# fransiskusbudi/multimodal_segmentation_project

Hardware: AMD Instinct MI355X
Metric: 3D volumes/sec (96^3, 4-class) fwd+bwd per node (higher is better)
Workload: dtype bf16; 1 GPU; UNet3D(1->4, features 16/32/64/128) 96^3 patch, per-GPU batch 2, fwd + Dice/CE loss + bwd + AdamW + metrics, dropout 0.0; global_batch=2, parallelism=dp1, hipgraph=False

## Files before the change

include/mi3d.h:

```cpp
#ifndef MI3D_H
#define MI3D_H
#include <stddef.h>
#include <stdint.h>

#ifdef __cplusplus
extern "C" {
#endif

#define MI3D_DTYPE_F32 0
#define MI3D_DTYPE_BF16 1
#define MI3D_MAX_LEVELS 6

const char* mi3d_last_error(void);
int mi3d_abi_version(void);

typedef struct mi3d_unet_desc {
    int32_t in_channels, out_channels;
    int32_t n_levels;
    int32_t features[MI3D_MAX_LEVELS];
    int32_t N, D, H, W;
    int32_t dtype;
    float bn_momentum, bn_eps;
} mi3d_unet_desc;

// ... 149 lines not shown
                 void* workspace, size_t workspace_bytes, void* stream);
int mi3d_fill_boxes_i64(int64_t* label, int C, int D, int H, int W, int n_holes, const int32_t* hole_lo,
                        const int32_t* hole_size, int64_t fill, void* stream);

size_t mi3d_conv3_workspace_bytes(int Cin, int Cout, int N, int D, int H, int W);
int mi3d_conv3_forward(int in_dtype, int out_dtype, const void* x, int xcs, int Cin, const float* w, const float* bias,
                       void* y, int ycs, int Cout, int N, int D, int H, int W, void* workspace, size_t workspace_bytes,
                       void* stream);
int mi3d_conv3_backward(int x_dtype, int dy_dtype, const void* x, int xcs, int Cin, const float* w, const void* dy,
                        int dycs, int Cout, void* dx, int dxcs, float* dW, float* db, int accumulate, int N, int D,
                        int H, int W, void* workspace, size_t workspace_bytes, void* stream);
size_t mi3d_bn_workspace_bytes(int C);
int mi3d_bn_relu_drop_forward(int dtype, const void* y, int ycs, int C, int64_t M, int64_t V, const float* gamma,
                              const float* beta, float* running_mean, float* running_var, int64_t* num_batches_tracked,
                              float momentum, float eps, int training, const float* drop, void* z, int zcs, float* stat,
                              void* workspace, void* stream);
int mi3d_bn_relu_drop_backward(int dtype, const void* dz, int dzcs, const void* y, int ycs, int C, int64_t M, int64_t V,
                               const float* stat, const float* drop, void* dy, int dycs, float* dgamma, float* dbeta,
                               int accumulate, void* workspace, void* stream);
int mi3d_bn_relu_drop_pool_forward(int dtype, const void* y, int ycs, int C, int N, int D, int H, int W, const float* gamma,
                                   const float* beta, float* running_mean, float* running_var, int64_t* num_batches_tracked,
                                   float momentum, float eps, const float* drop, void* z, int zcs, void* pooled, int pcs,
                                   float* stat, void* workspace, void* stream);
int mi3d_maxpool2_forward(int dtype, const void* z, int zcs, int C, int N, int D, int H, int W, void* p, int pcs,
                          void* stream);
int mi3d_maxpool2_backward(int dtype, const void* dp, int dpcs, const void* z, int zcs, const void* dskip, int dskipcs,
                           void* dz, int dzcs, int C, int N, int D, int H, int W, void* stream);
size_t mi3d_upconv2_workspace_bytes(int Cin, int Cout, int N, int D, int H, int W);
int mi3d_upconv2_forward(int dtype, const void* x, int xcs, int Cin, const float* w, const float* bias, void* y, int ycs,
                         int Cout, int N, int D, int H, int W, void* workspace, size_t workspace_bytes, void* stream);
int mi3d_upconv2_backward(int dtype, const void* x, int xcs, int Cin, const float* w, const void* gy, int gycs, int Cout,
                          void* dx, int dxcs, float* dW, float* db, int accumulate, int N, int D, int H, int W,
                          void* workspace, size_t workspace_bytes, void* stream);
size_t mi3d_conv1_workspace_bytes(int Cin, int Cout);
int mi3d_conv1_forward(int dtype, const void* z, int zcs, int Cin, const float* w, const float* bias, float* logits, int Cout,
                       int N, int64_t V, void* stream);
int mi3d_conv1_backward(int dtype, const void* z, int zcs, int Cin, const float* w, const float* dlogits, int Cout, void* dz,
                        int dzcs, float* dW, float* db, int accumulate, int N, int64_t V, void* workspace,
                        size_t workspace_bytes, void* stream);
int mi3d_ncdhw_to_ndhwc(int dtype, const float* src, void* dst, int dcs, int C, int N, int64_t V, void* stream);
int mi3d_ndhwc_to_ncdhw(int dtype, const void* src, int scs, float* dst, int C, int N, int64_t V, void* stream);

int mi3d_graph_begin(void* stream);
int mi3d_graph_end(void* stream, void** graph_exec_out);
int mi3d_graph_launch(void* graph_exec, void* stream);
int mi3d_graph_destroy(void* graph_exec);
// ... 6 lines not shown
```

multimodal_segmentation_project_amd/_lib.py:

```python
import contextlib
import ctypes as C
import os

import torch

_HERE = os.path.dirname(os.path.abspath(__file__))
LIB_PATH = os.environ.get("MI3D_LIB_PATH") or os.path.join(_HERE, "libmi3d.so")
MAX_LEVELS = 6
LOSS_COEF_FLOATS = 20
DTYPE_F32, DTYPE_BF16 = 0, 1

vp, i32, i64, f32, sz = C.c_void_p, C.c_int, C.c_int64, C.c_float, C.c_size_t


class UNetDesc(C.Structure):
    _fields_ = [("in_channels", C.c_int32), ("out_channels", C.c_int32), ("n_levels", C.c_int32),
                ("features", C.c_int32 * MAX_LEVELS), ("N", C.c_int32), ("D", C.c_int32), ("H", C.c_int32),
                ("W", C.c_int32), ("dtype", C.c_int32), ("bn_momentum", C.c_float), ("bn_eps", C.c_float)]


class LossCfg(C.Structure):
    _fields_ = [("w_ce", C.c_float), ("region_kind", C.c_int32), ("w_reg", C.c_float), ("alpha", C.c_float),
                ("beta", C.c_float), ("eps", C.c_float), ("w_kd", C.c_float), ("temperature", C.c_float)]

# ... 73 lines not shown
    "mi3d_preprocess_mri": (i32, [vp, vp, i64, f32, f32, vp, vp]),
    "mi3d_remap_labels": (i32, [vp, vp, i64, i32, vp]),
    "mi3d_zoom3_workspace_bytes": (sz, [i32, i32, i32]),
    "mi3d_zoom3_cubic": (i32, [vp, vp, i32, i32, i32, i32, i32, i32, vp, i32, vp, i32, vp, i32, i32, f32, f32, vp]),
    "mi3d_zoom3_nearest_i64": (i32, [vp, vp, i32, i32, i32, i32, i32, i32, vp, i32, vp, i32, vp, i32, vp]),
    "mi3d_reorient3": (i32, [vp, i32, vp, i32, i32, i32, i32, i64, i64, i64, i32, vp]),
    "mi3d_zoom3_cubic_src": (i32, [vp, i32, i64, i64, i64, vp, i32, i32, i32, i32, i32, i32, vp, i32, vp, i32, vp, i32, i32, f32, f32, vp]),
    "mi3d_zoom3_nearest_src": (i32, [vp, i32, i64, i64, i64, vp, i32, i32, i32, i32, i32, i32, vp, i32, vp, i32, vp, i32, vp]),
    "mi3d_merge_masks3": (i32, [_MP, i32, i64, i64, i64, vp, i32, i32, i32, i32, i32, i32, vp, i32, vp, i32, vp, i32, vp]),
    "mi3d_plane_affine": (i32, [vp, vp, vp, vp, i32, i32, i32, i32, i32, i32, C.POINTER(C.c_double), C.POINTER(C.c_double), i32, vp]),
    "mi3d_augment_workspace_bytes": (sz, []),
    "mi3d_augment": (i32, [vp, vp, vp, i32, i32, i32, i32, _AP, vp, sz, vp]),
    "mi3d_fill_boxes_i64": (i32, [vp, i32, i32, i32, i32, i32, C.POINTER(C.c_int32), C.POINTER(C.c_int32), i64, vp]),
    "mi3d_conv3_workspace_bytes": (sz, [i32, i32, i32, i32, i32, i32]),
    "mi3d_conv3_forward": (i32, [i32, i32, vp, i32, i32, vp, vp, vp, i32, i32, i32, i32, i32, i32, vp, sz, vp]),
    "mi3d_conv3_backward": (i32, [i32, i32, vp, i32, i32, vp, vp, i32, i32, vp, i32, vp, vp, i32, i32, i32, i32, i32,
                                  vp, sz, vp]),
    "mi3d_bn_workspace_bytes": (sz, [i32]),
    "mi3d_bn_relu_drop_forward": (i32, [i32, vp, i32, i32, i64, i64, vp, vp, vp, vp, vp, f32, f32, i32, vp, vp, i32,
                                        vp, vp, vp]),
    "mi3d_bn_relu_drop_backward": (i32, [i32, vp, i32, vp, i32, i32, i64, i64, vp, vp, vp, i32, vp, vp, i32, vp, vp]),
    "mi3d_bn_relu_drop_pool_forward": (i32, [i32, vp, i32, i32, i32, i32, i32, i32, vp, vp, vp, vp, vp, f32, f32, vp, vp, i32,
                                             vp, i32, vp, vp, vp]),
    "mi3d_conv1_workspace_bytes": (sz, [i32, i32]),
    "mi3d_conv1_forward": (i32, [i32, vp, i32, i32, vp, vp, vp, i32, i32, i64, vp]),
    "mi3d_conv1_backward": (i32, [i32, vp, i32, i32, vp, vp, i32, vp, i32, vp, vp, i32, i32, i64, vp, sz, vp]),
    "mi3d_maxpool2_forward": (i32, [i32, vp, i32, i32, i32, i32, i32, i32, vp, i32, vp]),
    "mi3d_maxpool2_backward": (i32, [i32, vp, i32, vp, i32, vp, i32, vp, i32, i32, i32, i32, i32, i32, vp]),
    "mi3d_upconv2_workspace_bytes": (sz, [i32, i32, i32, i32, i32, i32]),
    "mi3d_upconv2_forward": (i32, [i32, vp, i32, i32, vp, vp, vp, i32, i32, i32, i32, i32, i32, vp, sz, vp]),
    "mi3d_upconv2_backward": (i32, [i32, vp, i32, i32, vp, vp, i32, i32, vp, i32, vp, vp, i32, i32, i32, i32, i32, vp,
                                    sz, vp]),
    "mi3d_ncdhw_to_ndhwc": (i32, [i32, vp, vp, i32, i32, i32, i64, vp]),
    "mi3d_ndhwc_to_ncdhw": (i32, [i32, vp, i32, vp, i32, i32, i64, vp]),
    "mi3d_graph_begin": (i32, [vp]),
    "mi3d_graph_end": (i32, [vp, C.POINTER(vp)]),
    "mi3d_graph_launch": (i32, [vp, vp]),
    "mi3d_graph_destroy": (i32, [vp]),
}

_lib = None


class Mi3dError(RuntimeError):
    pass

# ... 82 lines not shown
```

multimodal_segmentation_project_amd/csrc/api.hip:

```cpp
#include "../../include/mi3d.h"
#include <stdlib.h>
#include <string.h>

#include "ops.h"

static_assert(MI3D_LOSS_COEF_FLOATS >= 2 * MI3D_MAX_CLASSES + 4, "coef buffer too small");

namespace {
struct RouteEntry { const char* name; int Mi3dRoutes::*field; };
const RouteEntry ROUTE_TABLE[] = {
#define MI3D_ROUTE_ENTRY(name, dflt) {#name, &Mi3dRoutes::name},
    MI3D_ROUTE_LIST(MI3D_ROUTE_ENTRY)
#undef MI3D_ROUTE_ENTRY
};
constexpr int N_ROUTES = sizeof(ROUTE_TABLE) / sizeof(ROUTE_TABLE[0]);
Mi3dRoutes load_routes() {
    Mi3dRoutes r;
    for (int i = 0; i < N_ROUTES; i++) {
        char env[64] = "MI3D_";
        size_t n = 5;
        for (const char* c = ROUTE_TABLE[i].name; *c && n + 1 < sizeof(env); c++) env[n++] = (*c >= 'a' && *c <= 'z') ? *c - 32 : *c;
        env[n] = 0;
        const char* v = getenv(env);
        if (!v) continue;
// ... 183 lines not shown
    BnSmall sm{(const float*)workspace, small_rows, gamma, beta, running_mean, running_var, num_batches_tracked, momentum, eps};
    return bn_apply_relu_drop(dtype, y, ycs, C, M, V, stat, drop, z, zcs, s, small_rows > 0 ? &sm : nullptr);
}
int mi3d_bn_relu_drop_backward(int dtype, const void* dz, int dzcs, const void* y, int ycs, int C, int64_t M, int64_t V,
                               const float* stat, const float* drop, void* dy, int dycs, float* dgamma, float* dbeta,
                               int accumulate, void* workspace, void* stream) {
    MI3D_CHECK_ARG(dz && y && stat && dy && workspace, "mi3d_bn_relu_drop_backward: null pointer");
    return bn_bwd(dtype, dz, dzcs, y, ycs, C, M, V, stat, drop, dy, dycs, dgamma, dbeta, accumulate, (float*)workspace,
                  (hipStream_t)stream);
}
int mi3d_bn_relu_drop_pool_forward(int dtype, const void* y, int ycs, int C, int N, int D, int H, int W, const float* gamma,
                                   const float* beta, float* running_mean, float* running_var, int64_t* num_batches_tracked,
                                   float momentum, float eps, const float* drop, void* z, int zcs, void* pooled, int pcs,
                                   float* stat, void* workspace, void* stream) {
    MI3D_CHECK_ARG(y && gamma && beta && z && pooled && stat && workspace, "mi3d_bn_relu_drop_pool_forward: null pointer");
    hipStream_t s = (hipStream_t)stream;
    Geo g{N, D, H, W};
    int small_rows = 0;
    MI3D_TRY(bn_train_stats(dtype, y, ycs, C, g.M(), gamma, beta, running_mean, running_var, num_batches_tracked, momentum, eps,
                            stat, (float*)workspace, s, &small_rows));
    BnSmall sm{(const float*)workspace, small_rows, gamma, beta, running_mean, running_var, num_batches_tracked, momentum, eps};
    return bn_apply_relu_drop_pool(dtype, y, ycs, C, g, stat, drop, z, zcs, pooled, pcs, s, small_rows > 0 ? &sm : nullptr);
}
size_t mi3d_conv1_workspace_bytes(int Cin, int Cout) { return conv1_bwd_ws_floats(Cin, Cout) * sizeof(float); }
int mi3d_conv1_forward(int dtype, const void* z, int zcs, int Cin, const float* w, const float* bias, float* logits, int Cout,
                       int N, int64_t V, void* stream) {
    MI3D_CHECK_ARG(z && w && logits, "mi3d_conv1_forward: null pointer");
    MI3D_CHECK_ARG(dtype == MI3D_F32 || dtype == MI3D_BF16, "mi3d_conv1_forward: bad dtype %d", dtype);
    return conv1_fwd(dtype, z, zcs, Cin, w, bias, logits, Cout, N, V, (hipStream_t)stream);
}
int mi3d_head_loss_supported(int dtype, int Cin, int C, const mi3d_loss_cfg* cfg) {
    return cfg && head_loss_bwd_ok(dtype, nullptr, Cin, Cin, C, to_cfg(cfg), nullptr, Cin) ? 1 : 0;
}
int mi3d_head_loss_forward(const void* z, int zcs, int Cin, const float* w, const float* bias, const int64_t* labels,
                           const float* teacher, int N, int C, int D, int64_t V, const mi3d_loss_cfg* cfg, float* loss_out, float* coef,
                           float* metrics_out, void* loss_workspace, void* metrics_workspace, float* logits_opt, void* stream) {
    MI3D_CHECK_ARG(z && w && labels && cfg && loss_out && coef && loss_workspace, "mi3d_head_loss_forward: null pointer");
    return head_loss_fwd(z, zcs, Cin, w, bias, labels, teacher, N, C, V, to_cfg(cfg), loss_out, coef, loss_workspace, (hipStream_t)stream,
                         D, metrics_out, metrics_workspace, logits_opt);
}
int mi3d_head_loss_backward(const void* z, int zcs, int Cin, const float* w, const float* bias, const int64_t* labels,
                            const float* teacher, int N, int C, int64_t V, const mi3d_loss_cfg* cfg, const float* coef,
                            const float* grad_scale, void* dz, int dzcs, float* dW, float* db, int accumulate, void* workspace,
                            size_t workspace_bytes, void* stream) {
    MI3D_CHECK_ARG(z && w && labels && cfg && coef && dz && workspace, "mi3d_head_loss_backward: null pointer");
    MI3D_CHECK_ARG(workspace_bytes >= mi3d_conv1_workspace_bytes(Cin, C), "mi3d_head_loss_backward: workspace too small");
// ... 149 lines not shown
```

multimodal_segmentation_project_amd/csrc/bn.hip:

```cpp
#include "ops.h"

namespace {

constexpr int BLK = 256;
constexpr int MAXBLK = 1024;
constexpr int FIN_T = 256;

template <int VEC> __device__ __forceinline__ bool row_map(int C, int& r, int& g, int& R) {
    int G = C / VEC;
    R = BLK / G;
    r = threadIdx.x / G;
    g = threadIdx.x - r * G;
    return r < R;
}

template <int VEC, int K> __device__ __forceinline__ void block_colreduce(const float (&acc)[K][VEC], int C, int r, int g, int R,
                                                                           bool active, float* lds, float* part) {
    if (active) {
#pragma unroll
        for (int k = 0; k < K; k++)
#pragma unroll
            for (int i = 0; i < VEC; i++) lds[((k * R + r) * C) + g * VEC + i] = acc[k][i];
    }
    __syncthreads();
// ... 197 lines not shown
        int c = threadIdx.x;
        if (c < C) {
            BnCoef k = bn_coef(sq[0], sq[1], t.M, t.gamma[c], t.beta[c], t.eps);
            ab[c] = k.a;
            ab[MAXC_BN + c] = k.b;
            if (blockIdx.x == 0)
                bn_publish(k, c, C, t.M, stat, t.running_mean, t.running_var, t.num_batches_tracked, t.momentum);
        }
        __syncthreads();
#pragma unroll
        for (int i = 0; i < VEC; i++) { a[i] = ab[g * VEC + i]; b[i] = ab[MAXC_BN + g * VEC + i]; }
    } else {
#pragma unroll
        for (int i = 0; i < VEC; i++) { a[i] = stat[2 * C + g * VEC + i]; b[i] = stat[3 * C + g * VEC + i]; }
    }
}

__device__ __forceinline__ float bn_act(float v, float a, float b, float s) {
    float t = fmaf(v, a, b);
    t = t > 0.f ? t : 0.f;
    return t * s;
}
__device__ __forceinline__ float bn_mask(float v, float a, float b, float s) { return fmaf(v, a, b) > 0.f ? s : 0.f; }

__global__ void bn_eval_stats_kernel(int C, const float* gamma, const float* beta, const float* rm,
                                     const float* rv, float eps, float* stat) {
    int c = blockIdx.x * blockDim.x + threadIdx.x;
    if (c >= C) return;
    double inv = 1.0 / sqrt((double)rv[c] + (double)eps);
    stat[c] = rm[c];
    stat[C + c] = (float)inv;
    stat[2 * C + c] = (float)((double)gamma[c] * inv);
    stat[3 * C + c] = (float)((double)beta[c] - (double)rm[c] * (double)gamma[c] * inv);
}

template <int VEC>
struct DropCache {
    float s[VEC];
    int64_t bound = 0;
    int smp = -1;
    __device__ __forceinline__ DropCache() {
#pragma unroll
        for (int i = 0; i < VEC; i++) s[i] = 1.f;
    }
    __device__ __forceinline__ void at(const float* __restrict__ drop, int64_t row, int64_t V, int C, int c0) {
        if (drop && row >= bound) {
// ... 312 lines not shown
        c2o = MAXC_BN;
    }
#pragma unroll
    for (int i = 0; i < VEC; i++) {
        int c = g * VEC + i;
        float mean = stat[c], inv = stat[C + c];
        a[i] = stat[2 * C + c]; b[i] = stat[3 * C + c];
        gg[i] = SMALL ? a[i] : coef[2 * C + c];
        bwd_coef(c12[c], c12[c2o + c], gg[i], mean, inv, A[i], B[i]);
    }
    DropCache<VEC> dc;
    for (; row < M; row += rstep) {
        float yv[VEC], gv[VEC], o[VEC];
        ldv<T, VEC>(y + row * ycs + g * VEC, yv);
        ldv<T, VEC>(dz + row * dzcs + g * VEC, gv);
        dc.at(drop, row, V, C, g * VEC);
#pragma unroll
        for (int i = 0; i < VEC; i++)
            o[i] = fmaf(gg[i] * bn_mask(yv[i], a[i], b[i], dc.s[i]), gv[i], fmaf(A[i], yv[i], B[i]));
        stv<T, VEC>(dy + row * dycs + g * VEC, o);
    }
}

__global__ void bn_fold_all_kernel(BnFoldJobs J) {
    const BnFoldJob& j = J.j[blockIdx.x];
    for (int c = threadIdx.x; c < j.C; c += blockDim.x) {
        double a = (double)j.gamma[c] / sqrt((double)j.rv[c] + (double)J.eps);
        j.scale[c] = (float)a;
        j.fbias[c] = (float)(((double)(j.conv_bias ? j.conv_bias[c] : 0.f) - (double)j.rm[c]) * a + (double)j.beta[c]);
    }
}

__global__ void bn_deferred_apply_kernel(BnDeferJobs J) {
    const BnDeferJob& j = J.j[blockIdx.x];
    for (int c = threadIdx.x; c < j.C; c += blockDim.x) {
        j.rm[c] = (float)((1.0 - J.momentum) * j.rm[c] + J.momentum * j.side[c]);
        j.rv[c] = (float)((1.0 - J.momentum) * j.rv[c] + J.momentum * j.side[j.C + c]);
    }
    if (threadIdx.x == 0 && j.nbt) *j.nbt += 1;
}

inline bool vec8_ok(int C, int cs_a, int cs_b, const void* pa, const void* pb, int esz) {
    return C % 8 == 0 && cs_a % 8 == 0 && cs_b % 8 == 0 && ((uintptr_t)pa % 16 == 0) && ((uintptr_t)pb % 16 == 0) &&
           (C / 8) <= BLK && esz > 0;
}

// ... 128 lines not shown
    DISPATCH_T(dtype, T, {
        bool v8 = vec8_ok(C, ycs, zcs, y, z, sizeof(T)) && pcs % 8 == 0 && ((uintptr_t)pooled % 16 == 0);
        int grid = v8 ? stream_grid(M / 8 * (C / 8), C / 8) : stream_grid(M / 8 * C, C);
        const T* yp = (const T*)y; T* zp = (T*)z; T* pp = (T*)pooled;
        const int G8 = C / 8;
        const bool pair = v8 && (G8 & (G8 - 1)) == 0 && G8 <= 32 && !mi3d_routes().no_pool_pair;
        if (pair) grid = stream_grid(M / 8 * G8 * 2, G8 * 2);
        if (small && small->nrows > SMALL_ROWS) {
            if (pair && dtype == MI3D_BF16 && wide_rows_ok(C, small->nrows)) {
                bn_apply_pool_wide_kernel<<<wide_grid(M / 8 * G8 * 2), WNT, 0, s>>>((const bf16*)y, ycs, C, g.N, g.D, g.H, g.W, stat, t, drop, (bf16*)z, zcs, (bf16*)pooled, pcs);
                MI3D_LAUNCH_CHECK();
                return 0;
            }
            MI3D_CHECK_ARG(small->nrows <= SMALL_ROWS, "bn_apply_pool: %d partial rows need the wide kernel (C = %d)", small->nrows, C);
        }
        DISPATCH_VEC(v8, VEC, DISPATCH_FLAG(small != nullptr, TRAIN, DISPATCH_FLAG(pair, PAIR, {
            bn_apply_pool_kernel<T, VEC, TRAIN, PAIR && VEC == 8><<<grid, BLK, 0, s>>>(yp, ycs, C, g.N, g.D, g.H, g.W, stat, t, drop, zp, zcs, pp, pcs);
        });););
        MI3D_LAUNCH_CHECK();
    });
    return 0;
}

int bn_bwd(int dtype, const void* dz, int dzcs, const void* y, int ycs, int C, int64_t M, int64_t V,
           const float* stat, const float* drop, void* dy, int dycs, float* dgamma, float* dbeta, int accumulate,
           float* ws, hipStream_t s, const SlabJob* extra, const float* skp, int ks, const SlabJob* extra2) {
    MI3D_CHECK_ARG(C >= 1 && C <= BLK && M >= 1, "bn_bwd: bad C=%d", C);
    MI3D_CHECK_ARG(!drop || M < (1ll << 32), "bn_bwd: dropout path needs M < 2^32 (32-bit sample index)");
    float* part = ws;
    float* coef = ws + (size_t)MAXBLK * 2 * C;
    bool small = bn_small(C, M);
    DISPATCH_T(dtype, T, {
        bool v8 = vec8_ok(C, ycs, dzcs, y, dz, sizeof(T)) && dycs % 8 == 0 && ((uintptr_t)dy % 16 == 0);
        MI3D_CHECK_ARG(!skp || (v8 && ks >= 1), "bn_bwd: split-K source needs the vector path");
        int G = v8 ? C / 8 : C, R = BLK / G;
        int nblk = reduce_grid(M, R);
        if (small) nblk = bn_small_rows(nblk);
        size_t lds = (size_t)2 * R * C * sizeof(float);
        const T* dzp = (const T*)dz; const T* yp = (const T*)y; T* dyp = (T*)dy;
        if (extra && extra->nblocks > 0) {
            SlabJob j2 = (extra2 && extra2->nblocks > 0) ? *extra2 : SlabJob();
            int tot = nblk + extra->nblocks + j2.nblocks;
            DISPATCH_VEC(v8, VEC, {
                bn_bwd_reduce_slab_kernel<T, VEC><<<tot, BLK, lds, s>>>(nblk, dzp, dzcs, yp, ycs, C, M, V, stat, drop, part, *extra, j2, skp, ks);
            });
        } else
            DISPATCH_VEC(v8, VEC, { bn_bwd_reduce_kernel<T, VEC><<<nblk, BLK, lds, s>>>(dzp, dzcs, yp, ycs, C, M, V, stat, drop, part, skp, ks); });
        MI3D_LAUNCH_CHECK();
        if (!small) {
            bn_bwd_finalize_kernel<<<C, FIN_T, 0, s>>>(part, nblk, C, M, stat, dgamma, dbeta, accumulate, coef);
            MI3D_LAUNCH_CHECK();
// ... 43 lines not shown
```

multimodal_segmentation_project_amd/csrc/ops.h:

```cpp
#pragma once
#include "common.h"
#include "slab_sum.h"

struct Geo {
    int N, D, H, W;
    int64_t V() const { return (int64_t)D * H * W; }
    int64_t M() const { return (int64_t)N * D * H * W; }
};

size_t conv3_direct_pack_floats(int Cin, int Cout);
int conv3_direct_pack(const float* w, int Cin, int Cout, float* wp_fwd, float* wp_dgrad, hipStream_t s,
                      const float* scale = nullptr);
int conv3_direct_fwd(int in_dtype, int out_dtype, const void* x, int xcs, int Cin, const float* wp,
                     const float* bias, void* y, int ycs, int Cout, Geo g, hipStream_t s, int relu = 0);
size_t conv3_direct_wgrad_ws_floats(int Cin, int Cout, Geo g);
int conv3_direct_wgrad(int x_dtype, int dy_dtype, const void* x, int xcs, int Cin, const void* dy, int dycs,
                       int Cout, Geo g, float* dW, float* db, int accumulate, float* ws, size_t ws_floats,
                       hipStream_t s);

bool conv3_mfma_supported(int Cin, int Cout, int xcs, int ycs);
size_t conv3_mfma_pack_elems(int Cin, int Cout);
int conv3_mfma_pack(const float* w, int Cin, int Cout, void* wp_fwd, void* wp_dgrad, Geo g, hipStream_t s);
struct PackJob { const float* w; void* a; void* b; int Cin, Cout, kind, mode_f, mode_d, blk0; const float* scale; };
constexpr int MAX_PACK_JOBS = 32;
// ... 45 lines not shown
struct BnSmall {
    const float* part; int nrows;
    const float* gamma; const float* beta; float* running_mean; float* running_var; int64_t* num_batches_tracked;
    float momentum, eps;
    int64_t M = 0;
};
int bn_train_finalize(const float* part, int nblk, int C, int64_t M, const float* gamma, const float* beta,
                      float* running_mean, float* running_var, int64_t* num_batches_tracked, float momentum,
                      float eps, float* stat, hipStream_t s);
int bn_eval_stats(int C, const float* gamma, const float* beta, const float* running_mean,
                  const float* running_var, float eps, float* stat, hipStream_t s);
struct BnFoldJob { const float* gamma; const float* beta; const float* rm; const float* rv; const float* conv_bias;
                   float* scale; float* fbias; int C; };
constexpr int MAX_FOLD_JOBS = 2 * (2 * 6 + 1);
struct BnFoldJobs { int n; float eps; BnFoldJob j[MAX_FOLD_JOBS]; };
int bn_fold_all(const BnFoldJobs& J, hipStream_t s);
struct BnDeferJob { float* rm; float* rv; int64_t* nbt; const double* side; int C; };
struct BnDeferJobs { int n; float momentum; BnDeferJob j[MAX_FOLD_JOBS]; };
int bn_deferred_apply(const BnDeferJobs& J, hipStream_t s);
int bn_apply_relu_drop(int dtype, const void* y, int ycs, int C, int64_t M, int64_t V, float* stat,
                       const float* drop, void* z, int zcs, hipStream_t s, const BnSmall* small = nullptr);
int bn_apply_relu_drop_pool(int dtype, const void* y, int ycs, int C, Geo g, float* stat, const float* drop, void* z, int zcs,
                            void* pooled, int pcs, hipStream_t s, const BnSmall* small = nullptr);
int bn_bwd(int dtype, const void* dz, int dzcs, const void* y, int ycs, int C, int64_t M, int64_t V,
           const float* stat, const float* drop, void* dy, int dycs, float* dgamma, float* dbeta,
           int accumulate, float* ws, hipStream_t s, const SlabJob* extra = nullptr, const float* skp = nullptr, int ks = 0,
           const SlabJob* extra2 = nullptr);
int slab_job_launch(const SlabJob& q, hipStream_t s);

int bn_train_stats_splitk(const float* skp, int ks, const float* bias, void* y, int ycs, int C, int64_t M, const float* gamma,
                          const float* beta, float* running_mean, float* running_var, int64_t* num_batches_tracked,
                          float momentum, float eps, float* stat, float* ws, hipStream_t s, int* small_rows = nullptr);

int maxpool2_fwd(int dtype, const void* z, int zcs, int C, Geo g, void* p, int pcs, hipStream_t s);
int maxpool2_bwd(int dtype, const void* dp, int dpcs, const void* z, int zcs, const void* dskip, int dskipcs,
                 void* dz, int dzcs, int C, Geo g, hipStream_t s, const float* skp = nullptr, int ks = 0);

int nearest_resize_fwd(int dtype, const void* x, int xcs, int C, Geo gi, void* y, int ycs, Geo go, hipStream_t s);
int nearest_resize_bwd(int dtype, const void* gy, int gycs, int C, Geo go, void* gx, int gxcs, Geo gi, hipStream_t s);

size_t upconv2_pack_floats(int Cin, int Cout);
int upconv2_pack(const float* w, int Cin, int Cout, float* wp_fwd, float* wp_bwd, hipStream_t s);
int upconv2_fwd(int dtype, const void* x, int xcs, int Cin, const float* wp_fwd, const float* bias, void* y,
                int ycs, int Cout, Geo g, hipStream_t s);
size_t upconv2_bwd_ws_floats(int Cin, int Cout, Geo g);
int upconv2_bwd(int dtype, const void* x, int xcs, int Cin, const void* gy, int gycs, int Cout,
                const float* wp_bwd, void* dx, int dxcs, float* dW, float* db, int accumulate, float* ws,
                size_t ws_floats, Geo g, hipStream_t s);

bool upconv2_mfma_supported(int Cin, int Cout, int xcs, int ycs);
// ... 65 lines not shown
```

multimodal_segmentation_project_amd/csrc/plan.hip:

```cpp
#include "../../include/mi3d.h"
#include <stdlib.h>

#include "ops.h"

namespace {

constexpr int MAXL = MI3D_MAX_LEVELS;

struct HalfP {
    int Cin, Cout;
    size_t y, stat, wpf, wpd;
    int pidx, bidx;
    int64_t drop_off;
    bool mfma;
    bool c1;
    int defer;
    size_t dyk;
};
struct BlockP {
    int level;
    HalfP h[2];
    size_t z1;
};
struct Plan {
// ... 328 lines not shown
        if (j.ev != c.waited_ev) { MI3D_HIP(hipStreamWaitEvent(c.s2, c.ev[j.ev % 3], 0)); c.waited_ev = j.ev; }
        const LayerIO v = layer_io(c, j.b, j.h, x);
        const HalfP& H = v.H;
        MI3D_TRY(conv3_mfma_wgrad(v.in, v.ics, H.Cin, c.at(H.dyk), H.Cout, H.Cout, v.g, (float*)grads[H.pidx], (float*)grads[H.pidx + 1],
                                  accumulate, c.at<float>(p.wgws3), p.wgws_floats, c.s2, v.ih, nullptr, j.wg_target));
        c.aux_used = true;
    }
    if (c.hq_head == c.nhq) c.hq_head = c.nhq = 0;
    return 0;
}

int flush_deferred(Ctx& c, const float* x, void* const* grads, int accumulate, bool lazy = false) {
    if (c.ndq == 0) return 0;
    MI3D_CHECK_ARG(c.nfork < 3, "flush_deferred: more than three forks in one call");
    const int e = c.nfork++;
    MI3D_HIP(hipEventRecord(c.ev[e % 3], c.s));
    for (int q = 0; q < c.ndq; q++) c.hq[c.nhq++] = Ctx::HJob{c.dq[q].b, c.dq[q].h, c.dq[q].wg_target, e};
    c.ndq = 0;
    if (!lazy) MI3D_TRY(drain_aux(c, x, grads, accumulate, -1));
    return 0;
}

int block_backward(Ctx& c, int b, const float* x, void* const* grads, const float* drop, const void* dz2,
                   int dzcs, void* dxin, int dxcs, int accumulate) {
    const Plan& p = c.p;
    auto G = [&](int i) { return grads ? (float*)grads[i] : nullptr; };
    const bool aux = c.s2 != nullptr && c.ev != nullptr;
    float* const skws = c.at<float>(p.skws);
    const float* dz_skp = nullptr;
    int dz_ks = 0;
    for (int h = 1; h >= 0; h--) {
        const LayerIO v = layer_io(c, b, h, x);
        const HalfP& H = v.H;
        const Geo g = v.g;
        int k = c.seq++;
        if (aux && c.nhq) MI3D_TRY(drain_aux(c, x, grads, accumulate, 3));
        const bool wg = G(H.pidx) || G(H.pidx + 1);
        const bool dfr = aux && H.defer && wg;
        void* dyb = dfr ? c.at(H.dyk) : c.at((k & 1) ? p.sB2 : p.sB);
        const void* dz = h == 1 ? dz2 : c.at(p.sC);
        int dcs = h == 1 ? dzcs : H.Cout;
        void* dx = h == 1 ? c.at(p.sC) : dxin;
        int dxs = h == 1 ? H.Cin : dxcs;
        auto dgrad = [&](int* ksd) {
            if (!H.mfma) return conv3_direct_fwd(p.dt, p.dt, dyb, H.Cout, H.Cout, c.at<float>(H.wpd), nullptr, dx, dxs, H.Cin, g, c.s);
            return conv3_mfma_fwd(dyb, H.Cout, H.Cout, c.at(H.wpd), nullptr, dx, dxs, H.Cin, g, nullptr, (dxs % 8 == 0) ? skws : nullptr,
                                  c.s, Halves(), v.ih, ksd, 0, CONV3_BWD_SPLITK_TARGET);
        };
        int ksd = 0;
        int* const ksp = (h == 1 || c.pool_defer) && dxs % 8 == 0 && !mi3d_routes().no_defer_tail ? &ksd : nullptr;
        auto file_partials = [&] {
            if (ksd > 0 && h == 1) { dz_skp = skws; dz_ks = ksd; }
            if (ksd > 0 && h == 0) c.pool_ks = ksd;
        };
        const SlabJob *extra, *extra2;
        c.pending.riders(extra, extra2);
        MI3D_TRY(bn_bwd(p.dt, dz, dcs, c.at(H.y), H.Cout, H.Cout, g.M(), g.V(), c.at<float>(H.stat),
                        drop ? drop + H.drop_off : nullptr, dyb, H.Cout, G(H.pidx + 2), G(H.pidx + 3), accumulate,
                        c.at<float>(p.bnws), c.s, extra, h == 0 ? dz_skp : nullptr, h == 0 ? dz_ks : 0, extra2));
        MI3D_TRY(c.pending.rode(c.s));
        if (dfr) {
            c.dq[c.ndq++] = Ctx::DJob{b, h, conv3_mfma_bwd_wg_target(H.Cin, H.Cout, v.ics, H.Cout, dx ? dxs : 8, g)};
        }
        if (aux)
            for (int q = 0; q < 2; q++)
                if (b == p.flush_b[q] && h == p.flush_h[q]) MI3D_TRY(flush_deferred(c, x, grads, accumulate, q == 1));
        if (dfr) {
            if (dx) { MI3D_TRY(dgrad(ksp)); file_partials(); }
            continue;
        }
        if (H.mfma && dx && wg && conv3_mfma_bwd_fused_persist_ok(H.Cin, H.Cout, v.ics, H.Cout, g)) {
            MI3D_TRY(conv3_mfma_bwd_fused_persist(v.in, v.ics, H.Cin, dyb, H.Cout, H.Cout, c.at(H.wpd), dx, dxs, g, G(H.pidx),
                                                  G(H.pidx + 1), accumulate, c.at<float>(p.wgws), p.wgws_floats, c.s, v.ih, v.ih,
                                                  c.pending.first(c.s)));
            continue;
        }
        if (H.mfma && dx && wg && !v.ih.on() && conv3_mfma_bwd_fused_ok(H.Cin, H.Cout, v.ics, H.Cout, dxs, g)) {
            MI3D_TRY(conv3_mfma_bwd_fused(v.in, v.ics, H.Cin, dyb, H.Cout, H.Cout, c.at(H.wpd), dx, dxs, g, G(H.pidx), G(H.pidx + 1),
                                          accumulate, c.at<float>(p.wgws), p.wgws_floats, skws, c.s, c.pending.first(c.s), ksp));
            file_partials();
            continue;
        }
// ... 336 lines not shown
            if (p.resize[l]) {
                MI3D_TRY(nearest_resize_bwd(p.dt, gup, gupcs, u.Cout, p.geo[l], c.at(p.uptmp), u.Cout, p.up_geo(l), c.s));
                gup = c.at(p.uptmp); gupcs = u.Cout;
            }
            if (p.up_mfma[i]) {
                SlabJob* ps = mi3d_routes().no_upbwd_carry ? nullptr : c.pending.carry();
                float* slabs = ps ? c.at<float>(p.wgws2) : wgws;
                if (!ps) ps = c.pending.first(c.s);
                MI3D_TRY(upconv2_mfma_bwd(u.in, u.Cin, u.Cin, gup, gupcs, u.Cout, u.w, c.at(p.gz[l + 1]), u.Cin, G(p.up_pidx(i)),
                                          G(p.up_pidx(i) + 1), accumulate, slabs, p.wgws_floats, u.g, c.s, ps));
            } else {
                c.pending.first(c.s);
                MI3D_TRY(upconv2_bwd(p.dt, u.in, u.Cin, u.Cin, gup, gupcs, u.Cout, u.wb, c.at(p.gz[l + 1]), u.Cin, G(p.up_pidx(i)),
                                     G(p.up_pidx(i) + 1), accumulate, wgws, p.wgws_floats, u.g, c.s));
            }
        } else if (seg == L + 1) {
            if (dgap)
                MI3D_TRY(gap_bwd(p.dt, dgap, gap_scale, c.at(p.gz[L]), p.C[L], p.C[L], d->N, p.geo[L].V(), dlogits ? 1 : 0, c.s));
            c.pool_defer = seg + 1 < seg_end && !mi3d_routes().no_pool_splitk;
            MI3D_TRY(block_backward(c, L, x, grads, drop_scales, c.at(p.gz[L]), p.C[L], c.at(p.gp[L - 1]), p.C[L - 1], accumulate));
            c.pool_defer = false;
        } else {
            int l = 2 * L + 1 - seg;
            MI3D_TRY(maxpool2_bwd(p.dt, c.at(p.gp[l]), p.C[l], c.at(p.cat[l]), p.catcs(l), dlogits ? c.at(p.gcat[l]) : nullptr,
                                  p.catcs(l), c.at(p.gz[l]), p.C[l], p.C[l], p.geo[l], c.s,
                                  c.pool_ks > 0 ? c.at<float>(p.skws) : nullptr, c.pool_ks));
            c.pool_ks = 0;
            void* dx = l > 0 ? c.at(p.gp[l - 1]) : nullptr;
            c.pool_defer = l > 0 && seg + 1 < seg_end && !mi3d_routes().no_pool_splitk;
            MI3D_TRY(block_backward(c, l, x, grads, drop_scales, c.at(p.gz[l]), p.C[l], dx, l > 0 ? p.C[l - 1] : 0, accumulate));
            c.pool_defer = false;
        }
    }
    MI3D_TRY(c.pending.finish(c.s));
    for (int i = 0; i < marks.n; i++)
        if (marks.seg[i] == seg_end - 1) MI3D_HIP(hipEventRecord(marks.ev[i], c.s));
    if (c.s2 && c.ev) {
        MI3D_TRY(flush_deferred(c, x, grads, accumulate));
        MI3D_TRY(drain_aux(c, x, grads, accumulate, -1));
    }
    if (c.aux_used) {
        MI3D_HIP(hipEventRecord(c.ev[3], c.s2));
        if (aux_join) MI3D_HIP(hipStreamWaitEvent(c.s, c.ev[3], 0));
    }
    return 0;
}

extern "C" {

int mi3d_unet_backward(const mi3d_unet_desc* d, const float* x, const void* const* params, void* const* grads,
                       const float* drop_scales, const float* dlogits, const float* dgap, float gap_scale, int accumulate,
                       int seg_begin, int seg_end, void* workspace, size_t workspace_bytes, void* stream, void* aux_stream,
                       void* const* events, int aux_join) {
// ... 17 lines not shown
```

Measured before the change: 979.7 volumes/s.

## Fuse MaxPool3d backward into BN-ReLU backward reduction kernel

Adds a fused kernel that recomputes the pooling argmax from the pre-BN activation and BN stats. It scatters the pooled gradient plus skip gradient into dz and accumulates the BN backward reductions in the same pass. The encoder backward path uses it instead of a separate maxpool2 backward launch whenever shape and alignment checks pass. This removes one kernel launch and one full read/write pass over dz at each encoder level. In exchange the reduction kernel does more arithmetic per element, and the argmax recompute must match the forward tie-breaking exactly.

Measured after the change: 988.1 volumes/s (median of 6 runs). No clear change (+0.9%).

```diff
diff --git a/include/mi3d.h b/include/mi3d.h
--- a/include/mi3d.h
+++ b/include/mi3d.h
@@ -195,6 +195,9 @@
                                    const float* beta, float* running_mean, float* running_var, int64_t* num_batches_tracked,
                                    float momentum, float eps, const float* drop, void* z, int zcs, void* pooled, int pcs,
                                    float* stat, void* workspace, void* stream);
+int mi3d_bn_relu_drop_pool_backward(int dtype, const void* dp, int dpcs, const void* dskip, int dskipcs, const void* y, int ycs,
+                                    int C, int N, int D, int H, int W, const float* stat, const float* drop, void* dz, int dzcs,
+                                    void* dy, int dycs, float* dgamma, float* dbeta, int accumulate, void* workspace, void* stream);
 int mi3d_maxpool2_forward(int dtype, const void* z, int zcs, int C, int N, int D, int H, int W, void* p, int pcs,
                           void* stream);
 int mi3d_maxpool2_backward(int dtype, const void* dp, int dpcs, const void* z, int zcs, const void* dskip, int dskipcs,
diff --git a/multimodal_segmentation_project_amd/_lib.py b/multimodal_segmentation_project_amd/_lib.py
--- a/multimodal_segmentation_project_amd/_lib.py
+++ b/multimodal_segmentation_project_amd/_lib.py
@@ -119,6 +119,8 @@
     "mi3d_bn_relu_drop_backward": (i32, [i32, vp, i32, vp, i32, i32, i64, i64, vp, vp, vp, i32, vp, vp, i32, vp, vp]),
     "mi3d_bn_relu_drop_pool_forward": (i32, [i32, vp, i32, i32, i32, i32, i32, i32, vp, vp, vp, vp, vp, f32, f32, vp, vp, i32,
                                              vp, i32, vp, vp, vp]),
+    "mi3d_bn_relu_drop_pool_backward": (i32, [i32, vp, i32, vp, i32, vp, i32, i32, i32, i32, i32, i32, vp, vp, vp, i32, vp, i32, vp,
+                                              vp, i32, vp, vp]),
     "mi3d_conv1_workspace_bytes": (sz, [i32, i32]),
     "mi3d_conv1_forward": (i32, [i32, vp, i32, i32, vp, vp, vp, i32, i32, i64, vp]),
     "mi3d_conv1_backward": (i32, [i32, vp, i32, i32, vp, vp, i32, vp, i32, vp, vp, i32, i32, i64, vp, sz, vp]),
diff --git a/multimodal_segmentation_project_amd/csrc/api.hip b/multimodal_segmentation_project_amd/csrc/api.hip
--- a/multimodal_segmentation_project_amd/csrc/api.hip
+++ b/multimodal_segmentation_project_amd/csrc/api.hip
@@ -229,6 +229,17 @@
     BnSmall sm{(const float*)workspace, small_rows, gamma, beta, running_mean, running_var, num_batches_tracked, momentum, eps};
     return bn_apply_relu_drop_pool(dtype, y, ycs, C, g, stat, drop, z, zcs, pooled, pcs, s, small_rows > 0 ? &sm : nullptr);
 }
+int mi3d_bn_relu_drop_pool_backward(int dtype, const void* dp, int dpcs, const void* dskip, int dskipcs, const void* y, int ycs,
+                                    int C, int N, int D, int H, int W, const float* stat, const float* drop, void* dz, int dzcs,
+                                    void* dy, int dycs, float* dgamma, float* dbeta, int accumulate, void* workspace, void* stream) {
+    MI3D_CHECK_ARG(dp && y && stat && dy && workspace, "mi3d_bn_relu_drop_pool_backward: null pointer");
+    const Geo g{N, D, H, W};
+    const PoolSrc ps{dp, dpcs, dskip, dskipcs, nullptr, 0, g};
+    MI3D_CHECK_ARG(bn_bwd_pool_ok(dtype, ps, dz, dzcs, y, ycs, C, dy, dycs),
+                   "mi3d_bn_relu_drop_pool_backward: no kernel for this shape, or bit 4 of route wide_bn is set (C=%d %dx%dx%d)", C, D, H, W);
+    return bn_bwd(dtype, dz, dzcs, y, ycs, C, g.M(), g.V(), stat, drop, dy, dycs, dgamma, dbeta, accumulate, (float*)workspace,
+                  (hipStream_t)stream, nullptr, nullptr, 0, nullptr, &ps);
+}
 size_t mi3d_conv1_workspace_bytes(int Cin, int Cout) { return conv1_bwd_ws_floats(Cin, Cout) * sizeof(float); }
 int mi3d_conv1_forward(int dtype, const void* z, int zcs, int Cin, const float* w, const float* bias, float* logits, int Cout,
                        int N, int64_t V, void* stream) {
diff --git a/multimodal_segmentation_project_amd/csrc/bn.hip b/multimodal_segmentation_project_amd/csrc/bn.hip
--- a/multimodal_segmentation_project_amd/csrc/bn.hip
+++ b/multimodal_segmentation_project_amd/csrc/bn.hip
@@ -243,6 +243,11 @@
     return t * s;
 }
 __device__ __forceinline__ float bn_mask(float v, float a, float b, float s) { return fmaf(v, a, b) > 0.f ? s : 0.f; }
+__device__ __forceinline__ float bn_act_pos(float v, float a, float b, float s, bool& pos) {
+    float t = fmaf(v, a, b);
+    pos = t > 0.f;
+    return (pos ? t : 0.f) * s;
+}
 
 __global__ void bn_eval_stats_kernel(int C, const float* gamma, const float* beta, const float* rm,
                                      const float* rv, float eps, float* stat) {
@@ -601,6 +606,139 @@
     }
 }
 
+struct PoolSrcK {
+    const bf16* dp; int dpcs;
+    const bf16* dskip; int dskipcs;
+    const float* skp; int ks;
+    int N, D, H, W;
+};
+typedef __attribute__((ext_vector_type(4))) unsigned u32x4;
+__device__ __forceinline__ bf16x8 ld16(const bf16* base, unsigned elem) {
+    return *reinterpret_cast<const bf16x8*>(reinterpret_cast<const char*>(base) + (size_t)(elem * 2u));
+}
+__device__ __forceinline__ void st16(bf16* base, unsigned elem, const float (&v)[8]) {
+    bf16x8 o;
+#pragma unroll
+    for (int i = 0; i < 8; i++) o[i] = (bf16)v[i];
+    *reinterpret_cast<bf16x8*>(reinterpret_cast<char*>(base) + (size_t)(elem * 2u)) = o;
+}
+__device__ __forceinline__ unsigned pool_key(float z, int k) {
+    const unsigned u = z == 0.f ? 0u : __float_as_uint(z);
+    const unsigned ord = (u & 0x80000000u) ? ~u : (u | 0x80000000u);
+    return z > -INFINITY ? ((ord & 0xffff0000u) | (unsigned)(7 - k)) : 0u;
+}
+__device__ __forceinline__ int pool_key_arg(unsigned key) { return key ? 7 - (int)(key & 15u) : 0; }
+template <bool SKIP, bool SPLITK, typename F>
+__device__ __forceinline__ void pool_dz_window(const PoolSrcK& ps, const bf16* __restrict__ y, int ycs, int C, int G, int g, int pc,
+                                               unsigned win, const PoolWin& pw, const float (&a)[8], const float (&b)[8],
+                                               const float (&s)[8], F&& each) {
+    const int base = pw.corner(ps.D, ps.H, ps.W) + pc;
+    int off[4];
+    bf16x8 yr[4], sk[4], gr;
+#pragma unroll
+    for (int q = 0; q < 4; q++) {
+        off[q] = base + tap_off(2 * q, ps.H, ps.W);
+        yr[q] = ld16(y, (unsigned)(off[q] * ycs + g * 8));
+    }
+#pragma unroll
+    for (int q = 0; q < 4; q++) {
+        if constexpr (SKIP) sk[q] = ld16(ps.dskip, (unsigned)(off[q] * ps.dskipcs + g * 8));
+        else {
+#pragma unroll
+            for (int i = 0; i < 8; i++) sk[q][i] = (bf16)0.f;
+        }
+    }
+    if constexpr (SPLITK) {
+        const int64_t Mp = (int64_t)ps.N * (ps.D / 2) * (ps.H / 2) * (ps.W / 2);
+        float gp[8];
+#pragma unroll
+        for (int i = 0; i < 8; i++) gp[i] = 0.f;
+        for (int k = 0; k < ps.ks; k++) {
+            const float* pp = ps.skp + ((int64_t)k * Mp + win) * C + g * 8;
+#pragma unroll
+            for (int i = 0; i < 8; i++) gp[i] += pp[i];
+        }
+#pragma unroll
+        for (int i = 0; i < 8; i++) gr[i] = (bf16)gp[i];
+    } else
+        gr = ld16(ps.dp, win * (unsigned)ps.dpcs + (unsigned)(g * 8));
+    unsigned key[8], pos = 0;
+#pragma unroll
+    for (int i = 0; i < 8; i++) key[i] = 0u;
+#pragma unroll
+    for (int q = 0; q < 4; q++) {
+#pragma unroll
+        for (int i = 0; i < 8; i++) {
+            bool p;
+            const float z = (float)(bf16)bn_act_pos((float)yr[q][i], a[i], b[i], s[i], p);
+            pos |= (p ? 1u : 0u) << (8 * q + i);
+            const unsigned kq = pool_key(z, 2 * q + pc);
+            key[i] = kq > key[i] ? kq : key[i];
+        }
+    }
+    int arg[8];
+#pragma unroll
+    for (int i = 0; i < 8; i++) {
+        const unsigned ok = (unsigned)__shfl_xor((int)key[i], G, 64);
+        arg[i] = pool_key_arg(ok > key[i] ? ok : key[i]);
+    }
+#pragma unroll
+    for (int q = 0; q < 4; q++) {
+        u32x4 t = __builtin_bit_cast(u32x4, yr[q]);
+        asm volatile("" : "+v"(t));
+        const bf16x8 yq = __builtin_bit_cast(bf16x8, t);
+        float o[8];
+#pragma unroll
+        for (int i = 0; i < 8; i++) {
+            o[i] = (float)sk[q][i];
+            o[i] += (arg[i] == 2 * q + pc) ? (float)gr[i] : 0.f;
+            o[i] = round_to<bf16>(o[i]);
+        }
+        each(off[q], yq, (pos >> (8 * q)) & 0xffu, o);
+    }
+}
+
+template <bool SKIP, bool SPLITK>
+__global__ __launch_bounds__(BLK) void pool_bn_bwd_reduce_kernel(int nred, PoolSrcK ps, const bf16* __restrict__ y, int ycs, int C,
+                                                                 const float* __restrict__ stat, const float* __restrict__ drop,
+                                                                 bf16* __restrict__ dz, int dzcs, float* __restrict__ part, SlabJob job,
+                                                                 SlabJob job2) {
+    if ((int)blockIdx.x >= nred) {
+        int bb = (int)blockIdx.x - nred;
+        if (bb < job.nblocks) slab_job_run(job, bb);
+        else slab_job_run(job2, bb - job.nblocks);
+        return;
+    }
+    extern __shared__ __attribute__((aligned(16))) float lds[];
+    int r, g, R;
+    row_map<8>(C, r, g, R);
+    const int G = C / 8, pc = r & 1;
+    const unsigned TPW = 2u * G, windows = (unsigned)ps.N * (ps.D / 2) * (ps.H / 2) * (ps.W / 2), wstep = ((unsigned)nred * BLK) / TPW;
+    float mean[8], inv[8], a[8], b[8], acc[2][8];
+#pragma unroll
+    for (int i = 0; i < 8; i++) {
+        mean[i] = stat[g * 8 + i]; inv[i] = stat[C + g * 8 + i];
+        a[i] = stat[2 * C + g * 8 + i]; b[i] = stat[3 * C + g * 8 + i];
+        acc[0][i] = acc[1][i] = 0.f;
+    }
+    DropCache<8> dc;
+    for (unsigned win = (blockIdx.x * BLK + threadIdx.x) / TPW; win < windows; win += wstep) {
+        const PoolWin pw(win, ps.D / 2, ps.H / 2, ps.W / 2);
+        dc.at_sample(drop, pw.n, C, g * 8);
+        pool_dz_window<SKIP, SPLITK>(ps, y, ycs, C, G, g, pc, win, pw, a, b, dc.s, [&](int off, const bf16x8& yq, unsigned pos, const float (&o)[8]) {
+            st16(dz, (unsigned)(off * dzcs + g * 8), o);
+#pragma unroll
+            for (int i = 0; i < 8; i++) {
+                const float yv = (float)yq[i];
+                float dyh = o[i] * ((pos >> i) & 1u ? dc.s[i] : 0.f);
+                acc[0][i] += dyh;
+                acc[1][i] += dyh * (yv - mean[i]) * inv[i];
+            }
+        });
+    }
+    block_colreduce<8, 2>(acc, C, r, g, R, true, lds, part);
+}
+
 __global__ void bn_fold_all_kernel(BnFoldJobs J) {
     const BnFoldJob& j = J.j[blockIdx.x];
     for (int c = threadIdx.x; c < j.C; c += blockDim.x) {
@@ -775,11 +913,62 @@
     return 0;
 }
 
+bool bn_bwd_pool_ok(int dtype, const PoolSrc& ps, const void* dz, int dzcs, const void* y, int ycs, int C, const void* dy, int dycs) {
+    const Geo g = ps.g;
+    const int G8 = C / 8;
+    auto al = [](const void* p) { return ((uintptr_t)p % 16) == 0; };
+    auto mx = [](int a, int b) { return a > b ? a : b; };
+    return !(mi3d_routes().wide_bn & 4) && dtype == MI3D_BF16 && C % 8 == 0 && (G8 & (G8 - 1)) == 0 && G8 >= 1 && G8 <= 32 &&
+           g.N >= 1 && g.D >= 2 && g.H >= 2 && g.W >= 2 && ((g.D | g.H | g.W) & 1) == 0 &&
+           g.M() * mx(mx(ycs, dzcs), mx(mx(dycs, ps.dskip ? ps.dskipcs : 0), mx(ps.dpcs, C))) < (1ll << 31) &&
+           ycs % 8 == 0 && dycs % 8 == 0 && ps.dpcs % 8 == 0 && (!ps.dskip || ps.dskipcs % 8 == 0) && al(y) && al(dy) && al(ps.dp) &&
+           al(ps.dskip) && dz && dzcs % 8 == 0 && al(dz) && (ps.ks > 0 ? ps.skp != nullptr : ps.dp != nullptr);
+}
+
+static int bn_bwd_pool(const PoolSrc& ps, void* dz, int dzcs, const void* y, int ycs, int C, int64_t M, const float* stat,
+                       const float* drop, void* dy, int dycs, float* dgamma, float* dbeta, int accumulate, float* ws, hipStream_t s,
+                       const SlabJob* extra, const SlabJob* extra2) {
+    float* part = ws;
+    float* coef = ws + (size_t)MAXBLK * 2 * C;
+    const bool small = bn_small(C, M);
+    const int G = C / 8, R = BLK / G;
+    const int64_t threads = M / 8 * G * 2;
+    int nblk = reduce_grid(M, R);
+    if (small) nblk = bn_small_rows(nblk);
+    if (nblk > cdiv(threads, BLK)) nblk = cdiv(threads, BLK);
+    const size_t lds = (size_t)2 * R * C * sizeof(float);
+    const PoolSrcK k{(const bf16*)ps.dp, ps.dpcs, (const bf16*)ps.dskip, ps.dskipcs, ps.ks > 0 ? ps.skp : nullptr, ps.ks,
+                     ps.g.N, ps.g.D, ps.g.H, ps.g.W};
+    const SlabJob j1 = (extra && extra->nblocks > 0) ? *extra : SlabJob();
+    const SlabJob j2 = (j1.nblocks > 0 && extra2 && extra2->nblocks > 0) ? *extra2 : SlabJob();
+    const int tot = nblk + j1.nblocks + j2.nblocks;
+    DISPATCH_FLAG(k.dskip != nullptr, SKIP, DISPATCH_FLAG(k.skp != nullptr, SPLITK, {
+        pool_bn_bwd_reduce_kernel<SKIP, SPLITK><<<tot, BLK, lds, s>>>(nblk, k, (const bf16*)y, ycs, C, stat, drop, (bf16*)dz, dzcs, part, j1, j2);
+    }););
+    MI3D_LAUNCH_CHECK();
+    if (!small) {
+        bn_bwd_finalize_kernel<<<C, FIN_T, 0, s>>>(part, nblk, C, M, stat, dgamma, dbeta, accumulate, coef);
+        MI3D_LAUNCH_CHECK();
+    }
+    DISPATCH_FLAG(small, SMALL, {
+        bn_bwd_apply_kernel<bf16, 8, SMALL><<<stream_grid(M * G, G), BLK, 0, s>>>((const bf16*)dz, dzcs, (const bf16*)y, ycs, C, M, ps.g.V(), stat,
+                                                                                 SMALL ? part : coef, nblk, dgamma, dbeta, accumulate, drop,
+                                                                                 (bf16*)dy, dycs);
+    });
+    MI3D_LAUNCH_CHECK();
+    return 0;
+}
+
 int bn_bwd(int dtype, const void* dz, int dzcs, const void* y, int ycs, int C, int64_t M, int64_t V,
            const float* stat, const float* drop, void* dy, int dycs, float* dgamma, float* dbeta, int accumulate,
-           float* ws, hipStream_t s, const SlabJob* extra, const float* skp, int ks, const SlabJob* extra2) {
+           float* ws, hipStream_t s, const SlabJob* extra, const float* skp, int ks, const SlabJob* extra2, const PoolSrc* pool) {
     MI3D_CHECK_ARG(C >= 1 && C <= BLK && M >= 1, "bn_bwd: bad C=%d", C);
     MI3D_CHECK_ARG(!drop || M < (1ll << 32), "bn_bwd: dropout path needs M < 2^32 (32-bit sample index)");
+    if (pool) {
+        MI3D_CHECK_ARG(!skp && pool->g.M() == M && pool->g.V() == V && bn_bwd_pool_ok(dtype, *pool, dz, dzcs, y, ycs, C, dy, dycs),
+                       "bn_bwd: no MaxPool3d-backward kernel for this shape (bn_bwd_pool_ok)");
+        return bn_bwd_pool(*pool, const_cast<void*>(dz), dzcs, y, ycs, C, M, stat, drop, dy, dycs, dgamma, dbeta, accumulate, ws, s, extra, extra2);
+    }
     float* part = ws;
     float* coef = ws + (size_t)MAXBLK * 2 * C;
     bool small = bn_small(C, M);
diff --git a/multimodal_segmentation_project_amd/csrc/ops.h b/multimodal_segmentation_project_amd/csrc/ops.h
--- a/multimodal_segmentation_project_amd/csrc/ops.h
+++ b/multimodal_segmentation_project_amd/csrc/ops.h
@@ -91,10 +91,17 @@
                        const float* drop, void* z, int zcs, hipStream_t s, const BnSmall* small = nullptr);
 int bn_apply_relu_drop_pool(int dtype, const void* y, int ycs, int C, Geo g, float* stat, const float* drop, void* z, int zcs,
                             void* pooled, int pcs, hipStream_t s, const BnSmall* small = nullptr);
+struct PoolSrc {
+    const void* dp; int dpcs;
+    const void* dskip; int dskipcs;
+    const float* skp; int ks;
+    Geo g;
+};
+bool bn_bwd_pool_ok(int dtype, const PoolSrc& ps, const void* dz, int dzcs, const void* y, int ycs, int C, const void* dy, int dycs);
 int bn_bwd(int dtype, const void* dz, int dzcs, const void* y, int ycs, int C, int64_t M, int64_t V,
            const float* stat, const float* drop, void* dy, int dycs, float* dgamma, float* dbeta,
            int accumulate, float* ws, hipStream_t s, const SlabJob* extra = nullptr, const float* skp = nullptr, int ks = 0,
-           const SlabJob* extra2 = nullptr);
+           const SlabJob* extra2 = nullptr, const PoolSrc* pool = nullptr);
 int slab_job_launch(const SlabJob& q, hipStream_t s);
 
 int bn_train_stats_splitk(const float* skp, int ks, const float* bias, void* y, int ycs, int C, int64_t M, const float* gamma,
diff --git a/multimodal_segmentation_project_amd/csrc/plan.hip b/multimodal_segmentation_project_amd/csrc/plan.hip
--- a/multimodal_segmentation_project_amd/csrc/plan.hip
+++ b/multimodal_segmentation_project_amd/csrc/plan.hip
@@ -374,7 +374,7 @@
 }
 
 int block_backward(Ctx& c, int b, const float* x, void* const* grads, const float* drop, const void* dz2,
-                   int dzcs, void* dxin, int dxcs, int accumulate) {
+                   int dzcs, void* dxin, int dxcs, int accumulate, const PoolSrc* pool = nullptr) {
     const Plan& p = c.p;
     auto G = [&](int i) { return grads ? (float*)grads[i] : nullptr; };
     const bool aux = c.s2 != nullptr && c.ev != nullptr;
@@ -409,7 +409,7 @@
         c.pending.riders(extra, extra2);
         MI3D_TRY(bn_bwd(p.dt, dz, dcs, c.at(H.y), H.Cout, H.Cout, g.M(), g.V(), c.at<float>(H.stat),
                         drop ? drop + H.drop_off : nullptr, dyb, H.Cout, G(H.pidx + 2), G(H.pidx + 3), accumulate,
-                        c.at<float>(p.bnws), c.s, extra, h == 0 ? dz_skp : nullptr, h == 0 ? dz_ks : 0, extra2));
+                        c.at<float>(p.bnws), c.s, extra, h == 0 ? dz_skp : nullptr, h == 0 ? dz_ks : 0, extra2, h == 1 ? pool : nullptr));
         MI3D_TRY(c.pending.rode(c.s));
         if (dfr) {
             c.dq[c.ndq++] = Ctx::DJob{b, h, conv3_mfma_bwd_wg_target(H.Cin, H.Cout, v.ics, H.Cout, dx ? dxs : 8, g)};
@@ -792,13 +792,18 @@
             c.pool_defer = false;
         } else {
             int l = 2 * L + 1 - seg;
-            MI3D_TRY(maxpool2_bwd(p.dt, c.at(p.gp[l]), p.C[l], c.at(p.cat[l]), p.catcs(l), dlogits ? c.at(p.gcat[l]) : nullptr,
-                                  p.catcs(l), c.at(p.gz[l]), p.C[l], p.C[l], p.geo[l], c.s,
-                                  c.pool_ks > 0 ? c.at<float>(p.skws) : nullptr, c.pool_ks));
+            const PoolSrc ps{c.at(p.gp[l]), p.C[l], dlogits ? c.at(p.gcat[l]) : nullptr, p.catcs(l),
+                             c.pool_ks > 0 ? c.at<float>(p.skws) : nullptr, c.pool_ks, p.geo[l]};
+            const HalfP& H1 = p.blk[l].h[1];
+            const bool fused = bn_bwd_pool_ok(p.dt, ps, c.at(p.gz[l]), p.C[l], c.at(H1.y), H1.Cout, p.C[l], c.at(p.sB), H1.Cout);
+            if (!fused)
+                MI3D_TRY(maxpool2_bwd(p.dt, ps.dp, ps.dpcs, c.at(p.cat[l]), p.catcs(l), ps.dskip, ps.dskipcs, c.at(p.gz[l]), p.C[l], p.C[l],
+                                      p.geo[l], c.s, ps.skp, ps.ks));
             c.pool_ks = 0;
             void* dx = l > 0 ? c.at(p.gp[l - 1]) : nullptr;
             c.pool_defer = l > 0 && seg + 1 < seg_end && !mi3d_routes().no_pool_splitk;
-            MI3D_TRY(block_backward(c, l, x, grads, drop_scales, c.at(p.gz[l]), p.C[l], dx, l > 0 ? p.C[l - 1] : 0, accumulate));
+            MI3D_TRY(block_backward(c, l, x, grads, drop_scales, c.at(p.gz[l]), p.C[l], dx, l > 0 ? p.C[l - 1] : 0, accumulate,
+                                    fused ? &ps : nullptr));
             c.pool_defer = false;
         }
     }
```
